# hyperconnect/TC-ResNet

Hardware: AMD Instinct MI355X
Metric: utterances/sec (1 s@16 kHz) TCResNet8-1.0 forward (higher is better)
Workload: dtype f32; 1 GPU; TCResNet8-1.0 eval forward, waveform->softmax, batch 4096/GPU, 49x40 MFCC (40/20 ms, FFT 1024), 12 classes; global_batch=4096, parallelism=dp1 (utterance shards, no collective)

## Files before the change

include/tcresnet_hip.h:

```cpp
#ifndef TCRESNET_HIP_H
#define TCRESNET_HIP_H

#include <stddef.h>
#include <stdint.h>

#ifdef __cplusplus
extern "C" {
#endif

#define TCR_ABI_VERSION 3
#define TCR_HALO 4
#define TCR_MAX_BLOCKS 16

typedef enum tcr_status {
    TCR_OK = 0,
    TCR_ERR_ARG = -1,
    TCR_ERR_HIP = -2,
    TCR_ERR_WORKSPACE = -3
} tcr_status;

int tcr_abi_version(void);
const char* tcr_last_error(void);
static inline int tcr_padded_len(int t) { return t + 2 * TCR_HALO; }

// ... 507 lines not shown
       TCR_TUNE_NET_SMALL = 27,
       TCR_TUNE_PW_POS = 28,
       TCR_TUNE_BN_APPLY = 29,
       TCR_TUNE_DW_DGRAD = 30,
       TCR_TUNE_DW_WGRAD = 31,
       TCR_TUNE_DW_FWD = 32,
       TCR_TUNE_WGRAD_PIPE = 33,
       TCR_TUNE_COMPOSE_RUN = 34,
       TCR_TUNE_COUNT = 35 };
int tcr_tune(int knob, int value);

int tcr_fused_deal_run(int nrt, int nt16, int nw, int wave, int* out3);

int tcr_fused_tm_taps(int k, int stride, int tin, int pad_lo, int tile, int* out2);
int tcr_fused_tm_deal(int k, int stride, int cin, int cout, int tin, int pad_lo, int nw, int wave, unsigned* jobs, int cap, int* mfma);
int tcr_net_fused_plan(const tcr_net* net, int batch, int* out, int cap);

void* tcr_internal_stream(int idx, void* caller_stream);

#ifdef __cplusplus
}
#endif
#endif
```

tc-resnet_amd/_lib.py:

```python
from __future__ import annotations

import ctypes as C
import os
from typing import Optional

HALO = 4
MAX_BLOCKS = 16
GRID_TILE = 256
MINE_TILE = 256
MINE_RADIUS_MAX = 2560
COMPOSE_TILE = 2048
REVERB_TILE = 4096
REVERB_STAGE = 1024
REVERB_TAPS_MAX = 16384
PHRASE_TILE = 256
PHRASE_MAX = 64
PHRASE_MAX_WORDS = 8
PHRASE_PRODUCT, PHRASE_MIN = 0, 1
DTW_MAX_TEMPLATES = 64
DTW_MAX_FEATURES = 64
ABI_VERSION = 3
_HERE = os.path.dirname(os.path.abspath(__file__))
HIP_LIB_PATH = os.path.join(_HERE, "lib", "libtcresnet_hip.so")

# ... 51 lines not shown
class TensorInfo(C.Structure):
    _fields_ = [("name", C.c_char * 96), ("kind", C.c_int32), ("arena", C.c_int32), ("offset", C.c_int64),
                ("size", C.c_int64), ("shape", C.c_int32 * 4), ("rank", C.c_int32)]


_P = C.c_void_p
_DTW_TABLES = (C.c_int, _P, _P, C.c_int, _P, _P, C.POINTER(DtwCfg))
_PROTOTYPES = {
    "tcr_abi_version": (C.c_int, []),
    "tcr_last_error": (C.c_char_p, []),
    "tcr_kernel_name": (C.c_char_p, [C.c_int]),
    "tcr_tune": (C.c_int, [C.c_int, C.c_int]),
    "tcr_fused_deal_run": (C.c_int, [C.c_int, C.c_int, C.c_int, C.c_int, C.POINTER(C.c_int)]),
    "tcr_fused_tm_taps": (C.c_int, [C.c_int, C.c_int, C.c_int, C.c_int, C.c_int, C.POINTER(C.c_int)]),
    "tcr_fused_tm_deal": (C.c_int, [C.c_int] * 8 + [C.POINTER(C.c_uint), C.c_int, C.POINTER(C.c_int)]),
    "tcr_net_fused_plan": (C.c_int, [_P, C.c_int, C.POINTER(C.c_int), C.c_int]),
    "tcr_internal_stream": (_P, [C.c_int, _P]),
    "tcr_frontend_resolve": (C.c_int, [C.POINTER(FrontendCfg)]),
    "tcr_frontend_plan_bytes": (C.c_size_t, [C.POINTER(FrontendCfg)]),
    "tcr_frontend_plan_init": (C.c_int, [C.POINTER(FrontendCfg), _P]),
    "tcr_frontend_plan_mel_matrix": (C.c_int, [C.POINTER(FrontendCfg), _P, _P]),
    "tcr_frontend_plan_dct_matrix": (C.c_int, [C.POINTER(FrontendCfg), _P, _P]),
    "tcr_frontend_fwd": (C.c_int, [C.POINTER(FrontendCfg), _P, _P, C.c_int, _P, _P]),
    "tcr_frontend_fwd_rounds": (C.c_int, [C.POINTER(FrontendCfg), _P, _P, C.c_int, _P, C.c_int, _P]),
    "tcr_features_to_planar": (C.c_int, [_P, C.c_int, C.c_int, C.c_int, _P, _P]),
    "tcr_features_from_planar": (C.c_int, [_P, C.c_int, C.c_int, C.c_int, _P, _P]),
    "tcr_tcresnet_create": (C.c_int, [C.POINTER(TCResNetCfg), C.POINTER(_P)]),
    "tcr_net_destroy": (None, [_P]),
    "tcr_net_param_floats": (C.c_int64, [_P]),
    "tcr_net_decay_floats": (C.c_int64, [_P]),
# ... 223 lines not shown
```

tc-resnet_amd/csrc/fused.hip:

```cpp
#include <cstdint>

#include "kernels.h"

namespace tcr {

typedef float f32x4 __attribute__((ext_vector_type(4)));
typedef float f32x2 __attribute__((ext_vector_type(2)));

__device__ __forceinline__ f32x4 buf_load_f32x4(buf_rsrc rs, unsigned lane_off_bytes, unsigned uniform_off_bytes) {
#if __has_builtin(__builtin_amdgcn_raw_buffer_load_b128)
    return __builtin_bit_cast(f32x4, __builtin_amdgcn_raw_buffer_load_b128(rs, (int)lane_off_bytes, (int)uniform_off_bytes, 0));
#else
    return (f32x4){buf_load_f32(rs, lane_off_bytes, uniform_off_bytes), buf_load_f32(rs, lane_off_bytes, uniform_off_bytes + 4u),
                   buf_load_f32(rs, lane_off_bytes, uniform_off_bytes + 8u), buf_load_f32(rs, lane_off_bytes, uniform_off_bytes + 12u)};
#endif
}
__device__ __forceinline__ f32x2 buf_load_f32x2(buf_rsrc rs, unsigned lane_off_bytes, unsigned uniform_off_bytes) {
#if __has_builtin(__builtin_amdgcn_raw_buffer_load_b64)
    return __builtin_bit_cast(f32x2, __builtin_amdgcn_raw_buffer_load_b64(rs, (int)lane_off_bytes, (int)uniform_off_bytes, 0));
#else
    return (f32x2){buf_load_f32(rs, lane_off_bytes, uniform_off_bytes), buf_load_f32(rs, lane_off_bytes, uniform_off_bytes + 4u)};
#endif
}

// ... 203 lines not shown
            for (int reg = 0; reg < 4; ++reg) {
                const int co = m * 16 + q * 4 + reg;
                if (co >= COUT) continue;
                float v = fmaf(ac[reg], sc[reg], sh[reg]);
                if (res) v = fmaxf(v + res[g * res_sz + co * TPO + kHalo + t], 0.f);
                else if (L.relu) v = fmaxf(v, 0.f);
                float* dst = yout + g * out_sz + co * TPO + kHalo + t;
                dst[0] = v;
                if (t == 0) { dst[-4] = 0.f; dst[-3] = 0.f; dst[-2] = 0.f; dst[-1] = 0.f; }
                if (t == TOUT - 1) { dst[1] = 0.f; dst[2] = 0.f; dst[3] = 0.f; dst[4] = 0.f; }
            }
        }
    }
}

template <int K, int S, int CIN, int COUT, int TIN, bool HAS_RES, int NTJ, bool WLDS, int AHEAD = 0, bool TM = false, int OCS = 0, bool IMG = false>
__device__ __forceinline__ void fused_job_s(const FusedArgs& a, const FusedLayer& L, const float* __restrict__ xin, const int in_sz,
                                            float* yout, const float* res, const float* w, const int npos, const int m, const int (&cc)[NTJ],
                                            const int r, const int q, const int jlo = 0, const int jhi = K - 1, const int wio = 0) {
    constexpr int TOUT = (TIN + S - 1) / S;
    constexpr int PADT = ((TOUT - 1) * S + K - TIN) > 0 ? ((TOUT - 1) * S + K - TIN) : 0;
    constexpr int PADLO = PADT / 2;
    constexpr int TPI = TM ? fused_tm_pitch(TIN, true, S) : TIN + 2 * kHalo;
    constexpr int TPO = TM ? fused_tm_pitch(TOUT, OCS != 0, OCS) : TOUT + 2 * kHalo;
    constexpr int TPR = TM ? fused_tm_pitch(TOUT, false, 0) : TPO;
    constexpr int JS = TM ? kTmGroup : 1;
    constexpr int C4 = CIN / 4;
    constexpr int WSTEP = 4 * COUT, XSTEP = 4 * TPI;
    const int out_sz = L.out_sz;
    const int res_sz = L.res_sz;
    const int ja = TM ? jlo : 0, jb = TM ? jhi : K - 1;
    int gg[NTJ], tt[NTJ];
    const float* xp[NTJ];
#pragma unroll
    for (int nt = 0; nt < NTJ; ++nt) {
        if constexpr (TM) {
            const int half = (TOUT % 2 == 1 && cc[nt] == TOUT / 2) ? 0 : (r >> 3);
            gg[nt] = half * 8 + min(r & 7, npos - 1);
            tt[nt] = cc[nt] * 16;
            xp[nt] = xin + q * TPI + (S == 1 ? gg[nt] : 2 * gg[nt] - (gg[nt] & 7)) + tt[nt] * S + kTmGroup * (kHalo - PADLO);
        } else {
        const int p = min(cc[nt], npos - 1);
        gg[nt] = p / TOUT;
        tt[nt] = p - gg[nt] * TOUT;
        xp[nt] = xin + gg[nt] * in_sz + q * TPI + tt[nt] * S + kHalo - PADLO;
        }
    }
    const float* wp = w + q * COUT + min(m * 16 + r, COUT - 1);
    static_assert(COUT % 4 == 0, "a lane's four output channels are valid or invalid together");
    const int cob = min(m * 16 + q * 4, COUT - 4);
    const buf_rsrc sr = make_rsrc(a.ss);
    const unsigned sl = (unsigned)cob * 4u;
    float sc[4], sh[4];
    if constexpr (IMG) {
        const f32x4 vs = buf_load_f32x4(sr, sl, (unsigned)L.ss_off * 4u), vh = buf_load_f32x4(sr, sl, (unsigned)(L.ss_off + L.c_pad) * 4u);
#pragma unroll
        for (int reg = 0; reg < 4; ++reg) { sc[reg] = vs[reg]; sh[reg] = vh[reg]; }
    } else {
#pragma unroll
    for (int reg = 0; reg < 4; ++reg) {
        sc[reg] = buf_load_f32(sr, sl, (unsigned)(L.ss_off + reg) * 4u);
        sh[reg] = buf_load_f32(sr, sl, (unsigned)(L.ss_off + L.c_pad + reg) * 4u);
    }
    }
    const buf_rsrc ir = make_rsrc(IMG ? a.wimg : a.params);
    const unsigned il = (unsigned)(q * 16 + r);
    const unsigned io = (unsigned)(kWimgHeader + wio + m * (K * C4 * 64)) * 4u;
    constexpr unsigned kTapBytes = (unsigned)(C4 * 64) * 4u;
    f32x4 acc[NTJ];
#pragma unroll
    for (int nt = 0; nt < NTJ; ++nt) acc[nt] = (f32x4){0.f, 0.f, 0.f, 0.f};
    if constexpr (AHEAD == 1) {
        const buf_rsrc wr = make_rsrc(a.params);
        const unsigned wl = (unsigned)(q * COUT + min(m * 16 + r, COUT - 1)) * 4u;
        const unsigned wo = (unsigned)L.w_off * 4u;
        float w0[C4], w1[C4];
        if constexpr (IMG) wimg_load<C4, 0, C4>(ir, il, io + (unsigned)ja * kTapBytes, w0);
        else {
#pragma unroll
        for (int c4 = 0; c4 < C4; ++c4) w0[c4] = buf_load_f32(wr, wl, wo + (unsigned)((ja * C4 + c4) * WSTEP) * 4u);
        }
        auto tap = [&](const int j, const float (&wu)[C4], float (&wf)[C4], const bool fill) {
            TCR_WHATIF_PRIO(32768, 2);
            if (fill && !(TCR_WHATIF(4096) && (!TCR_WHATIF(65536) || (S == 2 && CIN == 24 && COUT == 32)))) {
                if constexpr (IMG) wimg_load<C4, 0, C4>(ir, il, io + (unsigned)(j + 1) * kTapBytes, wf);
                else {
#pragma unroll
                for (int c4 = 0; c4 < C4; ++c4) wf[c4] = buf_load_f32(wr, wl, wo + (unsigned)(((j + 1) * C4 + c4) * WSTEP) * 4u);
                }
            }
            float b[NTJ][C4];
            if (TCR_WHATIF(8192) && j > 0) {
#pragma unroll
                for (int c4 = 0; c4 < C4; ++c4)
#pragma unroll
                    for (int nt = 0; nt < NTJ; ++nt) b[nt][c4] = wu[c4] + (float)nt;
            } else {
#pragma unroll
            for (int c4 = 0; c4 < C4; ++c4)
#pragma unroll
                for (int nt = 0; nt < NTJ; ++nt) b[nt][c4] = xp[nt][c4 * XSTEP + JS * j];
            }
            __builtin_amdgcn_sched_barrier(0);
            TCR_WHATIF_PRIO(16384, 2);
            TCR_WHATIF_PRIO(32768, 0);
#pragma unroll
            for (int c4 = 0; c4 < C4; ++c4)
#pragma unroll
                for (int nt = 0; nt < NTJ; ++nt) acc[nt] = TCR_MFMA(wu[c4], b[nt][c4], acc[nt]);
            TCR_WHATIF_PRIO(16384, 0);
        };
        if constexpr (TM) {
            int j = ja;
#pragma unroll 1
            for (; j + 2 <= jb; j += 2) {
                tap(j, w0, w1, true);
                tap(j + 1, w1, w0, true);
            }
            if (j == jb) {
                tap(j, w0, w1, false);
            } else {
                tap(j, w0, w1, true);
                tap(j + 1, w1, w0, false);
            }
// ... 38 lines not shown
    wfill_b(ja);
    constexpr int kTapUnroll = WLDS ? K : 1;
#pragma unroll kTapUnroll
    for (int j = ja; j <= jb; ++j) {
        const int jn = TCR_WHATIF(2) ? 0 : min(j + 1, jb);
        const int jx = TCR_WHATIF(4) ? 0 : JS * j;
        {
            float b[NTJ][H0 > 0 ? H0 : 1];
#pragma unroll
            for (int c4 = 0; c4 < H0; ++c4)
#pragma unroll
                for (int nt = 0; nt < NTJ; ++nt) b[nt][c4] = xp[nt][c4 * XSTEP + jx];
#pragma unroll
            for (int c4 = 0; c4 < H0; ++c4)
#pragma unroll
                for (int nt = 0; nt < NTJ; ++nt) acc[nt] = TCR_MFMA(wa[c4], b[nt][c4], acc[nt]);
            wfill_a(jn);
        }
        {
            float b[NTJ][H1];
#pragma unroll
            for (int c4 = 0; c4 < H1; ++c4)
#pragma unroll
                for (int nt = 0; nt < NTJ; ++nt) b[nt][c4] = xp[nt][(H0 + c4) * XSTEP + jx];
#pragma unroll
            for (int c4 = 0; c4 < H1; ++c4)
#pragma unroll
                for (int nt = 0; nt < NTJ; ++nt) acc[nt] = TCR_MFMA(wb[c4], b[nt][c4], acc[nt]);
            wfill_b(jn);
        }
    }
    }
    const int dump = a.buf_off[2] + a.group * a.buf_sz[2] + (q * 16 + r) - a.buf_off[L.out_buf];
    const float lo = L.relu ? 0.f : -3.4e38f;
    const bool cv = COUT % 16 == 0 || m * 16 + q * 4 < COUT;
    float rv[NTJ][4];
    if (HAS_RES) {
#pragma unroll
        for (int nt = 0; nt < NTJ; ++nt) {
            const int rb = TM ? cob * TPR + tt[nt] + gg[nt] : gg[nt] * res_sz + cob * TPO + kHalo + tt[nt];
#pragma unroll
            for (int reg = 0; reg < 4; ++reg) rv[nt][reg] = res[rb + reg * TPR];
        }
    }
#pragma unroll
    for (int nt = 0; nt < NTJ; ++nt) {
        const bool ok = (TM ? 2 * cc[nt] + (r >> 3) < TOUT && (r & 7) < npos : cc[nt] < npos) && cv && !TCR_WHATIF(32);
        const f32x4 ac = acc[nt];
        float* po = yout + (ok ? (TM ? tt[nt] + r + (OCS != 0 ? kTmGroup * kHalo : 0) : gg[nt] * out_sz + kHalo + tt[nt]) + cob * TPO : dump);
        const int pitch = ok ? TPO : 0;
#pragma unroll
        for (int reg = 0; reg < 4; ++reg) {
            float v = fmaf(ac[reg], sc[reg], sh[reg]);
            if (HAS_RES) v = fmaxf(v + rv[nt][reg], 0.f);
            else v = fmaxf(v, lo);
            *po = v;
            po += pitch;
        }
    }
}

template <int NW, int K, int S, int CIN, int COUT, int TIN, bool HAS_RES, int NTJ = 2, bool WLDS = false>
__device__ __forceinline__ void fused_layer_s(const FusedArgs& a, const FusedLayer& L, const float* __restrict__ xin, const int in_sz,
                                              float* lds, const int ng, const int wave, const int r_in, const int q_in,
                                              const int w_lds = 0) {
    const int oz = opaque_zero();
    const int r = r_in + oz, q = q_in + oz;
    constexpr int TOUT = (TIN + S - 1) / S;
    constexpr int NRT = (COUT + 15) / 16;
    constexpr int JP = 16 * NTJ;
    static_assert(CIN % 4 == 0, "channel quads");
    static_assert(NTJ == 1 || NTJ == 2 || NTJ == 4, "one, two or four 16-position tiles per job");
    float* yout = lds + a.buf_off[L.out_buf];
// ... 9 lines not shown
        for (int nt = 0; nt < NTJ; ++nt) cc[nt] = (IL && NTJ > 1) ? cp * JP + 32 * (nt >> 1) + 2 * r + (nt & 1) : cp * JP + 16 * nt + r;
        fused_job_s<K, S, CIN, COUT, TIN, HAS_RES, NTJ, WLDS>(a, L, xin, in_sz, yout, res, w, npos, m, cc, r, q);
    }
}

template <int NT, int COUT, int TOUT, int PITCH>
__device__ __forceinline__ void fused_zero_halo_tm(float* yout, const int tid_in) {
    if (TCR_WHATIF(1024)) return;
    const int tid = tid_in + opaque_zero();
    for (int i = tid; i < COUT * 16; i += NT) {
        float4* p = reinterpret_cast<float4*>(yout + (i >> 4) * PITCH + ((i & 8) ? kTmGroup * (kHalo + TOUT) : 0) + 4 * (i & 7));
        *p = make_float4(0.f, 0.f, 0.f, 0.f);
    }
}

template <int NW, int K, int S, int CIN, int COUT, int TIN, bool HAS_RES, int OCS, int AHEAD, bool IMG = false>
__device__ __forceinline__ void fused_layer_tm(const FusedArgs& a, const FusedLayer& L, float* lds, const int ng, const int wave, const int r_in, const int q_in, const int wio = 0) {
    constexpr int TOUT = (TIN + S - 1) / S;
    constexpr int PADT = ((TOUT - 1) * S + K - TIN) > 0 ? ((TOUT - 1) * S + K - TIN) : 0;
    static constexpr FusedTmDeal deal = fused_tm_deal(K, S, CIN, COUT, TIN, PADT / 2, NW);
    static_assert(fused_tm_deal_fits(deal, NW), "a wave's jobs exceed the deal's table (kTmMaxJobs)");
    float* yout = lds + a.buf_off[L.out_buf];
    if constexpr (OCS != 0) fused_zero_halo_tm<NW * 64, COUT, TOUT, fused_tm_pitch(TOUT, true, OCS)>(yout, (int)threadIdx.x);
    const int oz = opaque_zero();
    const int r = r_in + oz, q = q_in + oz;
    const float* xin = lds + a.buf_off[L.in_buf];
    const float* res = L.res_buf >= 0 ? lds + a.buf_off[L.res_buf] : nullptr;
    const float* w = a.params + L.w_off;
    const int n = deal.n[wave];
    for (int i = 0; i < n; ++i) {
        const unsigned jw = deal.job[wave][i];
        const int m = (int)(jw & 15u), c = (int)(jw >> 4 & 63u), lo = (int)(jw >> 11 & 15u), hi = (int)(jw >> 15 & 15u);
        if (jw >> 10 & 1u) {
            const int cc[2] = {c, c + 1};
            fused_job_s<K, S, CIN, COUT, TIN, HAS_RES, 2, false, AHEAD, true, OCS, IMG>(a, L, xin, 0, yout, res, w, ng, m, cc, r, q, lo, hi, wio);
        } else {
            const int cc[1] = {c};
            fused_job_s<K, S, CIN, COUT, TIN, HAS_RES, 1, false, AHEAD, true, OCS, IMG>(a, L, xin, 0, yout, res, w, ng, m, cc, r, q, lo, hi, wio);
        }
    }
}

template <int NW, int K, int S, int CIN, int COUT, int TIN, bool HAS_RES, int AHEAD = 0>
__device__ __forceinline__ void fused_layer_u(const FusedArgs& a, const FusedLayer& L, const float* __restrict__ xin, const int in_sz,
                                              float* lds, const int ng, const int wave, const int r_in, const int q_in) {
    const int oz = opaque_zero();
    const int r = r_in + oz, q = q_in + oz;
    constexpr int TOUT = (TIN + S - 1) / S;
    constexpr int NRT = (COUT + 15) / 16;
    constexpr bool IL = S == 1;
    float* yout = lds + a.buf_off[L.out_buf];
    const float* res = L.res_buf >= 0 ? lds + a.buf_off[L.res_buf] : nullptr;
    const int npos = ng * TOUT;
// ... 363 lines not shown
    }
}

struct Tc8Shape { int k, stride, cin, cout; };
__host__ __device__ constexpr Tc8Shape tc8_shape(const int li) {
    constexpr Tc8Shape shape[10] = {{3, 1, 40, 16}, {1, 2, 16, 24}, {9, 2, 16, 24}, {9, 1, 24, 24}, {1, 2, 24, 32},
                                    {9, 2, 24, 32}, {9, 1, 32, 32}, {1, 2, 32, 48}, {9, 2, 32, 48}, {9, 1, 48, 48}};
    return shape[li];
}
__host__ __device__ constexpr int tc8_wimg_off(const int li) {
    int n = 0;
    for (int i = 0; i < li && i < 10; ++i) n += wimg_layer_floats(tc8_shape(i).k, tc8_shape(i).cin, tc8_shape(i).cout);
    return n;
}

template <int NW, int T0, int WD, int NTJ0 = 2, bool TM = false>
__global__ __launch_bounds__(NW * 64) TCR_WAVES_PER_SIMD_4 void net_fused_tc8_kernel(const FusedArgs a) {
    constexpr bool IMG = false;
#include "fused_tc8_walk.inc"
}
template <int NW, int T0, int WD, int NTJ0, bool TM, bool IMG>
__device__ __forceinline__ void net_fused_tc8_walk(const FusedArgs& a) {
#include "fused_tc8_walk.inc"
}
template <int NW, int T0, int WD, int NTJ0, bool TM, bool WIMG>
__global__ __launch_bounds__(NW * 64) TCR_WAVES_PER_SIMD_4 void net_fused_tc8_kernel(const FusedArgs a) {
    static_assert(TM && WIMG, "the instance with a weight image is the time-major one");
    if (wimg_present(a)) net_fused_tc8_walk<NW, T0, WD, NTJ0, TM, true>(a);
    else net_fused_tc8_walk<NW, T0, WD, NTJ0, TM, false>(a);
}

template <int NW>
__device__ __forceinline__ void small_stage_weights(const float* __restrict__ src, int n_floats, float* dst, int wave, int lane) {
    for (int c0 = wave * 256; c0 < n_floats; c0 += NW * 256) {
        const int c = c0 + 4 * lane;
        if (c < n_floats) glds16(src + c, dst + c0);
    }
}

template <int NW, int T0>
__global__ __launch_bounds__(NW * 64) void net_small_tc8_kernel(const FusedArgs a, const int wa_off, const int wb_off) {
    constexpr int NT = NW * 64;
    constexpr int T1 = (T0 + 1) / 2, T2 = (T1 + 1) / 2, T3 = (T2 + 1) / 2;
    float* lds = reinterpret_cast<float*>(dyn_lds());
// ... 131 lines not shown
                                     {9, 1, 48, 48}, {9, 1, 48, 48}, {9, 1, 48, 48}, {1, 2, 48, 72}, {9, 2, 48, 72}, {9, 1, 72, 72}, {9, 1, 72, 72}, {9, 1, 72, 72}};
    if (a.n_layers != 16 || !a.in_global || a.in_c != 40) return 0;
    const int t0 = a.layer[0].tin;
    if (t0 != 49 && t0 != 98) return 0;
    int t = t0;
    for (int i = 0; i < 16; ++i) {
        const FusedLayer& L = a.layer[i];
        if (L.k != shape[i][0] || L.stride != shape[i][1] || L.cin != shape[i][2] || L.cout != shape[i][3] || L.tin != t) return 0;
        if (i == 2 || i == 7 || i == 12) t = (t + 1) / 2;
    }
    return t0;
}

static int fused_tc8_frames(const FusedArgs& a);
bool fused_tmajor_applies(const FusedArgs& a, const int waves) {
    return (tune_get(TCR_TUNE_NET_FUSED) == 0 || tune_get(TCR_TUNE_NET_FUSED) == 13) && a.group == kTmGroup && waves == 8 && a.nc == 12 && fused_tc8_frames(a) == 49;
}
static bool fused_tmajor_pitches_agree(const FusedArgs& a) {
    for (int i = 0; i < a.n_layers; ++i) {
        const FusedLayer& L = a.layer[i];
        const int ocs = (L.k == 1 || i == a.n_layers - 1) ? 0 : (L.stride == 2 ? 1 : 2);
        if (L.out_sz != fused_tm_pitch(L.tout, ocs != 0, ocs)) return false;
        if (i > 0 && L.in_sz != fused_tm_pitch(L.tin, true, L.stride)) return false;
        if (L.res_buf >= 0 && L.res_sz != fused_tm_pitch(L.tout, false, 0)) return false;
        if (L.pad_lo != (L.k == 9 ? 4 : L.k == 3 ? 1 : 0)) return false;
    }
    return a.feat_sz == fused_tm_pitch(a.feat_t, false, 0);
}

static int fused_tc8_frames(const FusedArgs& a) {
    if (a.n_layers != 10 || !a.in_global || a.in_c != 40) return 0;
// ... 221 lines not shown
    }
    const bool r2 = tune_get(TCR_TUNE_NET_FUSED) == 4;
    const bool j2 = tune_get(TCR_TUNE_NET_FUSED) == 8;
    const bool ju = tune_get(TCR_TUNE_NET_FUSED) == 9;
    const bool j4 = tune_get(TCR_TUNE_NET_FUSED) == 5;
    const bool jl = tune_get(TCR_TUNE_NET_FUSED) == 10;
    const bool jr = tune_get(TCR_TUNE_NET_FUSED) == 11;
#define TCR_FS(NW_, T_) if (tc8 == T_ && waves == NW_) kern = r2 ? net_fused_tc8_kernel<NW_, T_, -1> : (j4 ? net_fused_tc8_kernel<NW_, T_, 0, 4> : (ju ? net_fused_tc8_kernel<NW_, T_, 0, 0> : (j2 ? net_fused_tc8_kernel<NW_, T_, 0, 2> : ((jr || (T_ == 49 && !jl)) ? net_fused_tc8_kernel<NW_, T_, 0, 6> : net_fused_tc8_kernel<NW_, T_, 0, 3>))));
    TCR_FS(4, 49) TCR_FS(8, 49) TCR_FS(16, 49) TCR_FS(4, 98) TCR_FS(8, 98) TCR_FS(16, 98)
#undef TCR_FS
    if (a.tmajor) {
        if (!fused_tmajor_applies(a, waves) || !fused_tmajor_pitches_agree(a)) { set_error("fused kernel: time-major plan without its kernel instance"); return TCR_ERR_ARG; }
        constexpr int kImg = tc8_wimg_off(10);
        if (a.wimg_floats != kImg) { set_error("fused kernel: the plan's weight image has %d floats, the kernel's %d", a.wimg_floats, kImg); return TCR_ERR_ARG; }
        if (a.wimg && reinterpret_cast<uintptr_t>(a.wimg) % 16 != 0) { set_error("fused kernel: the frozen table's weight image is not on a 16-byte boundary"); return TCR_ERR_ARG; }
        kern = tune_get(TCR_TUNE_NET_FUSED) == 13 ? net_fused_tc8_kernel<8, 49, 0, 6, true> : net_fused_tc8_kernel<8, 49, 0, 6, true, true>;
    }
    const int tc14 = (kern || tune_get(TCR_TUNE_NET_FUSED) == 3 || tune_get(TCR_TUNE_NET_FUSED) == 4) ? 0 : fused_tc14w_frames(a);
#define TCR_F14(NW_, T_) if (tc14 == T_ && waves == NW_) kern = ju ? net_fused_tc14w_kernel<NW_, T_, 0> : (j2 ? net_fused_tc14w_kernel<NW_, T_, 2> : net_fused_tc14w_kernel<NW_, T_, 13>);
    TCR_F14(8, 49) TCR_F14(16, 49) TCR_F14(8, 98) TCR_F14(16, 98)
#undef TCR_F14
    if (kern) ring = 0;
#define TCR_FK(NW_, R_) if (!kern && waves == NW_ && ring == R_) kern = net_fused_kernel<NW_, R_>;
    TCR_FK(4, 4) TCR_FK(4, 8) TCR_FK(4, 16) TCR_FK(8, 4) TCR_FK(8, 8) TCR_FK(8, 16) TCR_FK(16, 4) TCR_FK(16, 8) TCR_FK(16, 16)
#undef TCR_FK
    if (!kern) { set_error("fused kernel: no instantiation for %d waves / ring %d", waves, ring); return TCR_ERR_ARG; }
    if (lds_bytes > 64 * 1024) {
        if (hipFuncSetAttribute(reinterpret_cast<const void*>(kern), hipFuncAttributeMaxDynamicSharedMemorySize, (int)lds_bytes) != hipSuccess) {
            (void)hipGetLastError();
            return 1;
        }
// ... 44 lines not shown

extern "C" int tcr_fused_tm_deal(int k, int stride, int cin, int cout, int tin, int pad_lo, int nw, int wave, unsigned* jobs, int cap, int* mfma) {
    if (!jobs || k < 1 || stride < 1 || cin < 4 || cout < 1 || cout > 256 || tin < 1 || tin > 126 || (nw != 4 && nw != 8 && nw != 16) || wave < 0 || wave >= nw || cap < tcr::kTmMaxJobs) {
        tcr::set_error("tcr_fused_tm_deal: bad arguments");
        return TCR_ERR_ARG;
    }
    const int tout = (tin + stride - 1) / stride;
    if (((cout + 15) / 16) * ((tout + 1) / 2) > nw * tcr::kTmMaxJobs) { tcr::set_error("tcr_fused_tm_deal: more jobs than the table holds"); return TCR_ERR_ARG; }
    const tcr::FusedTmDeal d = tcr::fused_tm_deal(k, stride, cin, cout, tin, pad_lo, nw);
    if (d.n[wave] > tcr::kTmMaxJobs) { tcr::set_error("tcr_fused_tm_deal: more jobs than the table holds"); return TCR_ERR_ARG; }
    for (int i = 0; i < d.n[wave]; ++i) jobs[i] = d.job[wave][i];
    if (mfma) *mfma = d.mfma;
    return d.n[wave];
}

extern "C" int tcr_fused_deal_run(int nrt, int nt16, int nw, int wave, int* out3) {
    if (!out3 || nrt < 1 || nt16 < 0 || nw < nrt || nw % nrt != 0 || wave < 0 || wave >= nw) {
        tcr::set_error("tcr_fused_deal_run: bad arguments (%d row tiles, %d column tiles, wave %d of %d)", nrt, nt16, wave, nw);
        return TCR_ERR_ARG;
    }
    const tcr::FusedRun run = tcr::fused_deal_run(nrt, nt16, nw, wave);
    out3[0] = run.m; out3[1] = run.c0; out3[2] = run.c1;
    return TCR_OK;
}
```

tc-resnet_amd/csrc/fused_tc8_walk.inc:

```
    constexpr int NT = NW * 64;
    constexpr int T1 = (T0 + 1) / 2, T2 = (T1 + 1) / 2;
    float* lds = reinterpret_cast<float*>(dyn_lds());
    const int tid = threadIdx.x;
    const int lane = tid & 63;
    const int wave = __builtin_amdgcn_readfirstlane(tid >> 6);
    const int r = lane & 15, q = lane >> 4;
    const int row = a.in_c * a.in_tp;
#if TCR_FUSED_WHATIF & 2048
    long long ts[14];
    int nts = 0;
#define TCR_TC8_BARRIER do { __syncthreads(); ts[nts++] = (long long)__builtin_readcyclecounter(); } while (0)
#elif TCR_FUSED_WHATIF & 8
#define TCR_TC8_BARRIER ((void)0)
#else
#define TCR_TC8_BARRIER __syncthreads()
#endif
    constexpr bool RES = WD >= 0 && NTJ0 == 6;
    constexpr int NTJU = RES ? 3 : NTJ0;
#define TCR_TC8_OCS(LI, K_, S_) ((K_ == 1 || LI == 9) ? 0 : (S_ == 2 ? 1 : 2))
#define TCR_TC8_WIO(LI) (IMG ? tc8_wimg_off(LI) : 0)
#define TCR_TC8(LI, K_, S_, CI_, CO_, T_) do { const FusedLayer& L_ = TCR_LAYER_ROW(WD >= 0, LI); \
        static_assert(tc8_shape(LI).k == K_ && tc8_shape(LI).stride == S_ && tc8_shape(LI).cin == CI_ && tc8_shape(LI).cout == CO_, "layer LI runs with row LI's shape (tc8_shape)"); \
        if constexpr (TM) fused_layer_tm<NW, K_, S_, CI_, CO_, T_, (LI == 3 || LI == 6 || LI == 9), TCR_TC8_OCS(LI, K_, S_), ((K_ == 9 && CI_ <= 32) ? 1 : 0), IMG>(a, L_, lds, ng, wave, r, q, TCR_TC8_WIO(LI)); \
        else fused_layer_sel<NW, K_, S_, CI_, CO_, T_, WD, (LI == 3 || LI == 6 || LI == 9), (K_ != 1 && LI != 9), ((LI >= 1 && LI <= 3 && NTJU == 4) ? 4 : (((NTJU == 0 || NTJU == 3) && K_ == 9) ? NTJU : 2))>(a, L_, lds + a.buf_off[L_.in_buf], L_.in_sz, lds, ng, wave, r, q); } while (0)
#define TCR_TC8_R(LI, S_, CI_, CO_, T_, WS_) do { const FusedLayer& L_ = TCR_LAYER_ROW(true, LI); \
        if constexpr (TM) fused_zero_halo_tm<NT, CO_, (T_ + S_ - 1) / S_, fused_tm_pitch((T_ + S_ - 1) / S_, true, TCR_TC8_OCS(LI, 9, S_))>(lds + a.buf_off[L_.out_buf], tid); \
        else fused_zero_halo<NT, CO_, (T_ + S_ - 1) / S_>(lds + a.buf_off[L_.out_buf], L_.out_sz, ng, tid); \
        fused_layer_r<NW, 9, S_, CI_, CO_, T_, (LI == 3), TM, TCR_TC8_OCS(LI, 9, S_), IMG>(a, L_, lds + a.buf_off[L_.in_buf], L_.in_sz, lds, ng, wave, r, q, WS_); } while (0)
    for (int grp = blockIdx.x; grp < (TCR_WHATIF(512) ? 0 : a.n_groups); grp += gridDim.x) {
        const int n0 = grp * a.group;
        const int ng = min(a.group, a.batch - n0);
#if TCR_FUSED_WHATIF & 2048
        nts = 0;
        ts[nts++] = (long long)__builtin_readcyclecounter();
#endif
        if constexpr (WD < 0) fused_layer_sel<NW, 3, 1, 40, 16, T0, WD, false>(a, a.layer[0], a.feat + (size_t)n0 * row, row, lds, ng, wave, r, q);
        else if (!TCR_WHATIF(64)) {
            const FusedLayer& L0 = TCR_LAYER_ROW(true, 0);
// ... 53 lines not shown
```

tc-resnet_amd/csrc/kernels.h:

```cpp
#pragma once
#include "tcr_common.h"

namespace tcr {

enum ConvEpilogue { EPI_RAW = 0, EPI_AFFINE = 1 };

struct ConvArgs {
    const float* x;
    const float* w;
    float* y;
    const float* scale;
    const float* shift;
    const float* res;
    int npos;
    int cin, cout;
    int tpi, tout, tpo;
    int xoff;
    int relu;
    int ostride, ooff;
    const float* add;
    const float* add_mask;
    int add_bcast;
};

// ... 189 lines not shown
        int best = -1;
        for (int i = 0; i < nj; ++i) if (!used[i] && (best < 0 || cost[i] > cost[best])) best = i;
        used[best] = true;
        int s = 0;
        for (int i = 1; i < 4 && i < nw; ++i) if (sload[i] < sload[s]) s = i;
        int w = s;
        for (int i = s + 4; i < nw; i += 4) if (wload[i] < wload[w]) w = i;
        if (d.n[w] < kTmMaxJobs) d.job[w][d.n[w]] = words[best];
        ++d.n[w];
        wload[w] += cost[best];
        sload[s] += cost[best];
    }
    return d;
}

struct FusedRun { int m, c0, c1; };
__host__ __device__ inline FusedRun fused_deal_run(const int nrt, const int nt16, const int nw, const int wave) {
    const int wpt = nw / nrt;
    const int m = wave / wpt, l = wave - m * wpt;
    const int per = nt16 / wpt, extra = nt16 - per * wpt;
    const int rank = (l + wpt - (m * extra) % wpt) % wpt;
    const int c0 = rank * per + (rank < extra ? rank : extra);
    return FusedRun{m, c0, c0 + per + (rank < extra ? 1 : 0)};
}

__host__ __device__ constexpr bool fused_tm_deal_fits(const FusedTmDeal& d, const int nw) {
    for (int w = 0; w < nw; ++w) if (d.n[w] > kTmMaxJobs) return false;
    return true;
}

// ... 342 lines not shown
```

Baseline: 20.63 million utterances/s.

## Span all output-channel row tiles per job in early tc8 layers

Adds a row-spanning job mode to the time-major fused tc8 kernel. For layers 1 and 2, each job computes every 16-channel output tile for a time column, so each activation B fragment loaded per tap is reused across all row tiles. A new deal function distributes these larger jobs across waves, and the default kernel selection now uses this mode. The trade is more accumulator and weight registers per lane and fewer, coarser jobs, which may unbalance waves or reduce occupancy.

Result: no change. 20.62 million utterances/s (-0.0%).

```diff
diff --git a/include/tcresnet_hip.h b/include/tcresnet_hip.h
--- a/include/tcresnet_hip.h
+++ b/include/tcresnet_hip.h
@@ -545,6 +545,7 @@
 
 int tcr_fused_tm_taps(int k, int stride, int tin, int pad_lo, int tile, int* out2);
 int tcr_fused_tm_deal(int k, int stride, int cin, int cout, int tin, int pad_lo, int nw, int wave, unsigned* jobs, int cap, int* mfma);
+int tcr_fused_tm_deal_rows(int k, int stride, int cin, int cout, int tin, int pad_lo, int nw, int ntj, int wave, unsigned* jobs, int cap, int* mfma);
 int tcr_net_fused_plan(const tcr_net* net, int batch, int* out, int cap);
 
 void* tcr_internal_stream(int idx, void* caller_stream);
diff --git a/tc-resnet_amd/_lib.py b/tc-resnet_amd/_lib.py
--- a/tc-resnet_amd/_lib.py
+++ b/tc-resnet_amd/_lib.py
@@ -89,6 +89,7 @@
     "tcr_fused_deal_run": (C.c_int, [C.c_int, C.c_int, C.c_int, C.c_int, C.POINTER(C.c_int)]),
     "tcr_fused_tm_taps": (C.c_int, [C.c_int, C.c_int, C.c_int, C.c_int, C.c_int, C.POINTER(C.c_int)]),
     "tcr_fused_tm_deal": (C.c_int, [C.c_int] * 8 + [C.POINTER(C.c_uint), C.c_int, C.POINTER(C.c_int)]),
+    "tcr_fused_tm_deal_rows": (C.c_int, [C.c_int] * 9 + [C.POINTER(C.c_uint), C.c_int, C.POINTER(C.c_int)]),
     "tcr_net_fused_plan": (C.c_int, [_P, C.c_int, C.POINTER(C.c_int), C.c_int]),
     "tcr_internal_stream": (_P, [C.c_int, _P]),
     "tcr_frontend_resolve": (C.c_int, [C.POINTER(FrontendCfg)]),
diff --git a/tc-resnet_amd/csrc/fused.hip b/tc-resnet_amd/csrc/fused.hip
--- a/tc-resnet_amd/csrc/fused.hip
+++ b/tc-resnet_amd/csrc/fused.hip
@@ -241,7 +241,7 @@
     }
 }
 
-template <int K, int S, int CIN, int COUT, int TIN, bool HAS_RES, int NTJ, bool WLDS, int AHEAD = 0, bool TM = false, int OCS = 0, bool IMG = false>
+template <int K, int S, int CIN, int COUT, int TIN, bool HAS_RES, int NTJ, bool WLDS, int AHEAD = 0, bool TM = false, int OCS = 0, bool IMG = false, int MT = 1>
 __device__ __forceinline__ void fused_job_s(const FusedArgs& a, const FusedLayer& L, const float* __restrict__ xin, const int in_sz,
                                             float* yout, const float* res, const float* w, const int npos, const int m, const int (&cc)[NTJ],
                                             const int r, const int q, const int jlo = 0, const int jhi = K - 1, const int wio = 0) {
@@ -254,6 +254,7 @@
     constexpr int JS = TM ? kTmGroup : 1;
     constexpr int C4 = CIN / 4;
     constexpr int WSTEP = 4 * COUT, XSTEP = 4 * TPI;
+    static_assert(MT == 1 || (TM && AHEAD == 1 && !WLDS), "row-spanning jobs: the time-major walk with a tap of weight lookahead");
     const int out_sz = L.out_sz;
     const int res_sz = L.res_sz;
     const int ja = TM ? jlo : 0, jb = TM ? jhi : K - 1;
@@ -275,53 +276,61 @@
     }
     const float* wp = w + q * COUT + min(m * 16 + r, COUT - 1);
     static_assert(COUT % 4 == 0, "a lane's four output channels are valid or invalid together");
-    const int cob = min(m * 16 + q * 4, COUT - 4);
     const buf_rsrc sr = make_rsrc(a.ss);
-    const unsigned sl = (unsigned)cob * 4u;
-    float sc[4], sh[4];
+    int cob[MT];
+    float sc[MT][4], sh[MT][4];
+#pragma unroll
+    for (int mt = 0; mt < MT; ++mt) {
+    cob[mt] = min((m + mt) * 16 + q * 4, COUT - 4);
+    const unsigned sl = (unsigned)cob[mt] * 4u;
     if constexpr (IMG) {
         const f32x4 vs = buf_load_f32x4(sr, sl, (unsigned)L.ss_off * 4u), vh = buf_load_f32x4(sr, sl, (unsigned)(L.ss_off + L.c_pad) * 4u);
 #pragma unroll
-        for (int reg = 0; reg < 4; ++reg) { sc[reg] = vs[reg]; sh[reg] = vh[reg]; }
+        for (int reg = 0; reg < 4; ++reg) { sc[mt][reg] = vs[reg]; sh[mt][reg] = vh[reg]; }
     } else {
 #pragma unroll
     for (int reg = 0; reg < 4; ++reg) {
-        sc[reg] = buf_load_f32(sr, sl, (unsigned)(L.ss_off + reg) * 4u);
-        sh[reg] = buf_load_f32(sr, sl, (unsigned)(L.ss_off + L.c_pad + reg) * 4u);
+        sc[mt][reg] = buf_load_f32(sr, sl, (unsigned)(L.ss_off + reg) * 4u);
+        sh[mt][reg] = buf_load_f32(sr, sl, (unsigned)(L.ss_off + L.c_pad + reg) * 4u);
+    }
     }
     }
     const buf_rsrc ir = make_rsrc(IMG ? a.wimg : a.params);
     const unsigned il = (unsigned)(q * 16 + r);
     const unsigned io = (unsigned)(kWimgHeader + wio + m * (K * C4 * 64)) * 4u;
-    constexpr unsigned kTapBytes = (unsigned)(C4 * 64) * 4u;
-    f32x4 acc[NTJ];
-#pragma unroll
-    for (int nt = 0; nt < NTJ; ++nt) acc[nt] = (f32x4){0.f, 0.f, 0.f, 0.f};
+    constexpr unsigned kTapBytes = (unsigned)(C4 * 64) * 4u, kRowBytes = (unsigned)K * kTapBytes;
+    f32x4 acc[NTJ][MT];
+#pragma unroll
+    for (int nt = 0; nt < NTJ; ++nt)
+#pragma unroll
+        for (int mt = 0; mt < MT; ++mt) acc[nt][mt] = (f32x4){0.f, 0.f, 0.f, 0.f};
     if constexpr (AHEAD == 1) {
         const buf_rsrc wr = make_rsrc(a.params);
-        const unsigned wl = (unsigned)(q * COUT + min(m * 16 + r, COUT - 1)) * 4u;
+        unsigned wl[MT];
+#pragma unroll
+        for (int mt = 0; mt < MT; ++mt) wl[mt] = (unsigned)(q * COUT + min((m + mt) * 16 + r, COUT - 1)) * 4u;
         const unsigned wo = (unsigned)L.w_off * 4u;
-        float w0[C4], w1[C4];
-        if constexpr (IMG) wimg_load<C4, 0, C4>(ir, il, io + (unsigned)ja * kTapBytes, w0);
-        else {
-#pragma unroll
-        for (int c4 = 0; c4 < C4; ++c4) w0[c4] = buf_load_f32(wr, wl, wo + (unsigned)((ja * C4 + c4) * WSTEP) * 4u);
-        }
-        auto tap = [&](const int j, const float (&wu)[C4], float (&wf)[C4], const bool fill) {
+        float w0[MT][C4], w1[MT][C4];
+        auto wreq = [&](const int j, float (&wf)[MT][C4]) {
+#pragma unroll
+            for (int mt = 0; mt < MT; ++mt) {
+                if constexpr (IMG) wimg_load<C4, 0, C4>(ir, il, io + (unsigned)mt * kRowBytes + (unsigned)j * kTapBytes, wf[mt]);
+                else {
+#pragma unroll
+                for (int c4 = 0; c4 < C4; ++c4) wf[mt][c4] = buf_load_f32(wr, wl[mt], wo + (unsigned)((j * C4 + c4) * WSTEP) * 4u);
+                }
+            }
+        };
+        wreq(ja, w0);
+        auto tap = [&](const int j, const float (&wu)[MT][C4], float (&wf)[MT][C4], const bool fill) {
             TCR_WHATIF_PRIO(32768, 2);
-            if (fill && !(TCR_WHATIF(4096) && (!TCR_WHATIF(65536) || (S == 2 && CIN == 24 && COUT == 32)))) {
-                if constexpr (IMG) wimg_load<C4, 0, C4>(ir, il, io + (unsigned)(j + 1) * kTapBytes, wf);
-                else {
-#pragma unroll
-                for (int c4 = 0; c4 < C4; ++c4) wf[c4] = buf_load_f32(wr, wl, wo + (unsigned)(((j + 1) * C4 + c4) * WSTEP) * 4u);
-                }
-            }
+            if (fill && !(TCR_WHATIF(4096) && (!TCR_WHATIF(65536) || (S == 2 && CIN == 24 && COUT == 32)))) wreq(j + 1, wf);
             float b[NTJ][C4];
             if (TCR_WHATIF(8192) && j > 0) {
 #pragma unroll
                 for (int c4 = 0; c4 < C4; ++c4)
 #pragma unroll
-                    for (int nt = 0; nt < NTJ; ++nt) b[nt][c4] = wu[c4] + (float)nt;
+                    for (int nt = 0; nt < NTJ; ++nt) b[nt][c4] = wu[0][c4] + (float)nt;
             } else {
 #pragma unroll
             for (int c4 = 0; c4 < C4; ++c4)
@@ -334,7 +343,9 @@
 #pragma unroll
             for (int c4 = 0; c4 < C4; ++c4)
 #pragma unroll
-                for (int nt = 0; nt < NTJ; ++nt) acc[nt] = TCR_MFMA(wu[c4], b[nt][c4], acc[nt]);
+                for (int nt = 0; nt < NTJ; ++nt)
+#pragma unroll
+                    for (int mt = 0; mt < MT; ++mt) acc[nt][mt] = TCR_MFMA(wu[mt][c4], b[nt][c4], acc[nt][mt]);
             TCR_WHATIF_PRIO(16384, 0);
         };
         if constexpr (TM) {
@@ -403,7 +414,7 @@
 #pragma unroll
             for (int c4 = 0; c4 < H0; ++c4)
 #pragma unroll
-                for (int nt = 0; nt < NTJ; ++nt) acc[nt] = TCR_MFMA(wa[c4], b[nt][c4], acc[nt]);
+                for (int nt = 0; nt < NTJ; ++nt) acc[nt][0] = TCR_MFMA(wa[c4], b[nt][c4], acc[nt][0]);
             wfill_a(jn);
         }
         {
@@ -415,19 +426,21 @@
 #pragma unroll
             for (int c4 = 0; c4 < H1; ++c4)
 #pragma unroll
-                for (int nt = 0; nt < NTJ; ++nt) acc[nt] = TCR_MFMA(wb[c4], b[nt][c4], acc[nt]);
+                for (int nt = 0; nt < NTJ; ++nt) acc[nt][0] = TCR_MFMA(wb[c4], b[nt][c4], acc[nt][0]);
             wfill_b(jn);
         }
     }
     }
     const int dump = a.buf_off[2] + a.group * a.buf_sz[2] + (q * 16 + r) - a.buf_off[L.out_buf];
     const float lo = L.relu ? 0.f : -3.4e38f;
-    const bool cv = COUT % 16 == 0 || m * 16 + q * 4 < COUT;
+#pragma unroll
+    for (int mt = 0; mt < MT; ++mt) {
+    const bool cv = COUT % 16 == 0 || (m + mt) * 16 + q * 4 < COUT;
     float rv[NTJ][4];
     if (HAS_RES) {
 #pragma unroll
         for (int nt = 0; nt < NTJ; ++nt) {
-            const int rb = TM ? cob * TPR + tt[nt] + gg[nt] : gg[nt] * res_sz + cob * TPO + kHalo + tt[nt];
+            const int rb = TM ? cob[mt] * TPR + tt[nt] + gg[nt] : gg[nt] * res_sz + cob[mt] * TPO + kHalo + tt[nt];
 #pragma unroll
             for (int reg = 0; reg < 4; ++reg) rv[nt][reg] = res[rb + reg * TPR];
         }
@@ -435,17 +448,18 @@
 #pragma unroll
     for (int nt = 0; nt < NTJ; ++nt) {
         const bool ok = (TM ? 2 * cc[nt] + (r >> 3) < TOUT && (r & 7) < npos : cc[nt] < npos) && cv && !TCR_WHATIF(32);
-        const f32x4 ac = acc[nt];
-        float* po = yout + (ok ? (TM ? tt[nt] + r + (OCS != 0 ? kTmGroup * kHalo : 0) : gg[nt] * out_sz + kHalo + tt[nt]) + cob * TPO : dump);
+        const f32x4 ac = acc[nt][mt];
+        float* po = yout + (ok ? (TM ? tt[nt] + r + (OCS != 0 ? kTmGroup * kHalo : 0) : gg[nt] * out_sz + kHalo + tt[nt]) + cob[mt] * TPO : dump);
         const int pitch = ok ? TPO : 0;
 #pragma unroll
         for (int reg = 0; reg < 4; ++reg) {
-            float v = fmaf(ac[reg], sc[reg], sh[reg]);
+            float v = fmaf(ac[reg], sc[mt][reg], sh[mt][reg]);
             if (HAS_RES) v = fmaxf(v + rv[nt][reg], 0.f);
             else v = fmaxf(v, lo);
             *po = v;
             po += pitch;
         }
+    }
     }
 }
 
@@ -485,11 +499,13 @@
     }
 }
 
-template <int NW, int K, int S, int CIN, int COUT, int TIN, bool HAS_RES, int OCS, int AHEAD, bool IMG = false>
+template <int NW, int K, int S, int CIN, int COUT, int TIN, bool HAS_RES, int OCS, int AHEAD, bool IMG = false, int ROWS = 0>
 __device__ __forceinline__ void fused_layer_tm(const FusedArgs& a, const FusedLayer& L, float* lds, const int ng, const int wave, const int r_in, const int q_in, const int wio = 0) {
     constexpr int TOUT = (TIN + S - 1) / S;
     constexpr int PADT = ((TOUT - 1) * S + K - TIN) > 0 ? ((TOUT - 1) * S + K - TIN) : 0;
-    static constexpr FusedTmDeal deal = fused_tm_deal(K, S, CIN, COUT, TIN, PADT / 2, NW);
+    constexpr int MT = ROWS != 0 ? (COUT + 15) / 16 : 1;
+    static_assert(ROWS == 0 || AHEAD == 1, "row-spanning jobs walk with a tap of weight lookahead");
+    static constexpr FusedTmDeal deal = ROWS != 0 ? fused_tm_deal_rows(K, S, CIN, COUT, TIN, PADT / 2, NW, ROWS) : fused_tm_deal(K, S, CIN, COUT, TIN, PADT / 2, NW);
     static_assert(fused_tm_deal_fits(deal, NW), "a wave's jobs exceed the deal's table (kTmMaxJobs)");
     float* yout = lds + a.buf_off[L.out_buf];
     if constexpr (OCS != 0) fused_zero_halo_tm<NW * 64, COUT, TOUT, fused_tm_pitch(TOUT, true, OCS)>(yout, (int)threadIdx.x);
@@ -502,12 +518,12 @@
     for (int i = 0; i < n; ++i) {
         const unsigned jw = deal.job[wave][i];
         const int m = (int)(jw & 15u), c = (int)(jw >> 4 & 63u), lo = (int)(jw >> 11 & 15u), hi = (int)(jw >> 15 & 15u);
-        if (jw >> 10 & 1u) {
+        if (ROWS != 1 && (jw >> 10 & 1u)) {
             const int cc[2] = {c, c + 1};
-            fused_job_s<K, S, CIN, COUT, TIN, HAS_RES, 2, false, AHEAD, true, OCS, IMG>(a, L, xin, 0, yout, res, w, ng, m, cc, r, q, lo, hi, wio);
+            fused_job_s<K, S, CIN, COUT, TIN, HAS_RES, 2, false, AHEAD, true, OCS, IMG, MT>(a, L, xin, 0, yout, res, w, ng, m, cc, r, q, lo, hi, wio);
         } else {
             const int cc[1] = {c};
-            fused_job_s<K, S, CIN, COUT, TIN, HAS_RES, 1, false, AHEAD, true, OCS, IMG>(a, L, xin, 0, yout, res, w, ng, m, cc, r, q, lo, hi, wio);
+            fused_job_s<K, S, CIN, COUT, TIN, HAS_RES, 1, false, AHEAD, true, OCS, IMG, MT>(a, L, xin, 0, yout, res, w, ng, m, cc, r, q, lo, hi, wio);
         }
     }
 }
@@ -901,20 +917,25 @@
     return n;
 }
 
+__host__ __device__ constexpr int tc8_rows_policy(const int rs, const int li) {
+    return (rs == 1 && (li == 1 || li == 2)) ? 1 : 0;
+}
+
 template <int NW, int T0, int WD, int NTJ0 = 2, bool TM = false>
 __global__ __launch_bounds__(NW * 64) TCR_WAVES_PER_SIMD_4 void net_fused_tc8_kernel(const FusedArgs a) {
     constexpr bool IMG = false;
+    constexpr int RS = 0;
 #include "fused_tc8_walk.inc"
 }
-template <int NW, int T0, int WD, int NTJ0, bool TM, bool IMG>
+template <int NW, int T0, int WD, int NTJ0, bool TM, bool IMG, int RS>
 __device__ __forceinline__ void net_fused_tc8_walk(const FusedArgs& a) {
 #include "fused_tc8_walk.inc"
 }
-template <int NW, int T0, int WD, int NTJ0, bool TM, bool WIMG>
+template <int NW, int T0, int WD, int NTJ0, bool TM, bool WIMG, int RS = 0>
 __global__ __launch_bounds__(NW * 64) TCR_WAVES_PER_SIMD_4 void net_fused_tc8_kernel(const FusedArgs a) {
     static_assert(TM && WIMG, "the instance with a weight image is the time-major one");
-    if (wimg_present(a)) net_fused_tc8_walk<NW, T0, WD, NTJ0, TM, true>(a);
-    else net_fused_tc8_walk<NW, T0, WD, NTJ0, TM, false>(a);
+    if (wimg_present(a)) net_fused_tc8_walk<NW, T0, WD, NTJ0, TM, true, RS>(a);
+    else net_fused_tc8_walk<NW, T0, WD, NTJ0, TM, false, RS>(a);
 }
 
 template <int NW>
@@ -1076,7 +1097,7 @@
 
 static int fused_tc8_frames(const FusedArgs& a);
 bool fused_tmajor_applies(const FusedArgs& a, const int waves) {
-    return (tune_get(TCR_TUNE_NET_FUSED) == 0 || tune_get(TCR_TUNE_NET_FUSED) == 13) && a.group == kTmGroup && waves == 8 && a.nc == 12 && fused_tc8_frames(a) == 49;
+    return (tune_get(TCR_TUNE_NET_FUSED) == 0 || tune_get(TCR_TUNE_NET_FUSED) == 13 || tune_get(TCR_TUNE_NET_FUSED) == 14) && a.group == kTmGroup && waves == 8 && a.nc == 12 && fused_tc8_frames(a) == 49;
 }
 static bool fused_tmajor_pitches_agree(const FusedArgs& a) {
     for (int i = 0; i < a.n_layers; ++i) {
@@ -1328,7 +1349,8 @@
         constexpr int kImg = tc8_wimg_off(10);
         if (a.wimg_floats != kImg) { set_error("fused kernel: the plan's weight image has %d floats, the kernel's %d", a.wimg_floats, kImg); return TCR_ERR_ARG; }
         if (a.wimg && reinterpret_cast<uintptr_t>(a.wimg) % 16 != 0) { set_error("fused kernel: the frozen table's weight image is not on a 16-byte boundary"); return TCR_ERR_ARG; }
-        kern = tune_get(TCR_TUNE_NET_FUSED) == 13 ? net_fused_tc8_kernel<8, 49, 0, 6, true> : net_fused_tc8_kernel<8, 49, 0, 6, true, true>;
+        const int knob = tune_get(TCR_TUNE_NET_FUSED);
+        kern = knob == 13 ? net_fused_tc8_kernel<8, 49, 0, 6, true> : (knob == 14 ? net_fused_tc8_kernel<8, 49, 0, 6, true, true> : net_fused_tc8_kernel<8, 49, 0, 6, true, true, 1>);
     }
     const int tc14 = (kern || tune_get(TCR_TUNE_NET_FUSED) == 3 || tune_get(TCR_TUNE_NET_FUSED) == 4) ? 0 : fused_tc14w_frames(a);
 #define TCR_F14(NW_, T_) if (tc14 == T_ && waves == NW_) kern = ju ? net_fused_tc14w_kernel<NW_, T_, 0> : (j2 ? net_fused_tc14w_kernel<NW_, T_, 2> : net_fused_tc14w_kernel<NW_, T_, 13>);
@@ -1403,6 +1425,19 @@
     return d.n[wave];
 }
 
+extern "C" int tcr_fused_tm_deal_rows(int k, int stride, int cin, int cout, int tin, int pad_lo, int nw, int ntj, int wave, unsigned* jobs, int cap, int* mfma) {
+    if (!jobs || k < 1 || stride < 1 || cin < 4 || cout < 1 || cout > 256 || tin < 1 || tin > 126 || (nw != 4 && nw != 8 && nw != 16) || (ntj != 1 && ntj != 2) || wave < 0 ||
+        wave >= nw || cap < tcr::kTmMaxJobs) {
+        tcr::set_error("tcr_fused_tm_deal_rows: bad arguments");
+        return TCR_ERR_ARG;
+    }
+    const tcr::FusedTmDeal d = tcr::fused_tm_deal_rows(k, stride, cin, cout, tin, pad_lo, nw, ntj);
+    if (!tcr::fused_tm_deal_fits(d, nw)) { tcr::set_error("tcr_fused_tm_deal_rows: more jobs than the table holds"); return TCR_ERR_ARG; }
+    for (int i = 0; i < d.n[wave]; ++i) jobs[i] = d.job[wave][i];
+    if (mfma) *mfma = d.mfma;
+    return d.n[wave];
+}
+
 extern "C" int tcr_fused_deal_run(int nrt, int nt16, int nw, int wave, int* out3) {
     if (!out3 || nrt < 1 || nt16 < 0 || nw < nrt || nw % nrt != 0 || wave < 0 || wave >= nw) {
         tcr::set_error("tcr_fused_deal_run: bad arguments (%d row tiles, %d column tiles, wave %d of %d)", nrt, nt16, wave, nw);
diff --git a/tc-resnet_amd/csrc/fused_tc8_walk.inc b/tc-resnet_amd/csrc/fused_tc8_walk.inc
--- a/tc-resnet_amd/csrc/fused_tc8_walk.inc
+++ b/tc-resnet_amd/csrc/fused_tc8_walk.inc
@@ -21,7 +21,7 @@
 #define TCR_TC8_WIO(LI) (IMG ? tc8_wimg_off(LI) : 0)
 #define TCR_TC8(LI, K_, S_, CI_, CO_, T_) do { const FusedLayer& L_ = TCR_LAYER_ROW(WD >= 0, LI); \
         static_assert(tc8_shape(LI).k == K_ && tc8_shape(LI).stride == S_ && tc8_shape(LI).cin == CI_ && tc8_shape(LI).cout == CO_, "layer LI runs with row LI's shape (tc8_shape)"); \
-        if constexpr (TM) fused_layer_tm<NW, K_, S_, CI_, CO_, T_, (LI == 3 || LI == 6 || LI == 9), TCR_TC8_OCS(LI, K_, S_), ((K_ == 9 && CI_ <= 32) ? 1 : 0), IMG>(a, L_, lds, ng, wave, r, q, TCR_TC8_WIO(LI)); \
+        if constexpr (TM) fused_layer_tm<NW, K_, S_, CI_, CO_, T_, (LI == 3 || LI == 6 || LI == 9), TCR_TC8_OCS(LI, K_, S_), (((K_ == 9 && CI_ <= 32) || tc8_rows_policy(RS, LI) != 0) ? 1 : 0), IMG, tc8_rows_policy(RS, LI)>(a, L_, lds, ng, wave, r, q, TCR_TC8_WIO(LI)); \
         else fused_layer_sel<NW, K_, S_, CI_, CO_, T_, WD, (LI == 3 || LI == 6 || LI == 9), (K_ != 1 && LI != 9), ((LI >= 1 && LI <= 3 && NTJU == 4) ? 4 : (((NTJU == 0 || NTJU == 3) && K_ == 9) ? NTJU : 2))>(a, L_, lds + a.buf_off[L_.in_buf], L_.in_sz, lds, ng, wave, r, q); } while (0)
 #define TCR_TC8_R(LI, S_, CI_, CO_, T_, WS_) do { const FusedLayer& L_ = TCR_LAYER_ROW(true, LI); \
         if constexpr (TM) fused_zero_halo_tm<NT, CO_, (T_ + S_ - 1) / S_, fused_tm_pitch((T_ + S_ - 1) / S_, true, TCR_TC8_OCS(LI, 9, S_))>(lds + a.buf_off[L_.out_buf], tid); \
diff --git a/tc-resnet_amd/csrc/kernels.h b/tc-resnet_amd/csrc/kernels.h
--- a/tc-resnet_amd/csrc/kernels.h
+++ b/tc-resnet_amd/csrc/kernels.h
@@ -227,6 +227,44 @@
     return d;
 }
 
+__host__ __device__ constexpr FusedTmDeal fused_tm_deal_rows(const int k, const int stride, const int cin, const int cout, const int tin, const int pad_lo, const int nw,
+                                                             const int ntj) {
+    FusedTmDeal d{};
+    const int tout = (tin + stride - 1) / stride, nt16 = (tout + 1) / 2, nrt = (cout + 15) / 16;
+    unsigned words[64] = {};
+    int cost[64] = {};
+    int nj = 0;
+    for (int c = 0; c < nt16;) {
+        const FusedTaps t = fused_tm_taps(k, stride, tin, pad_lo, c);
+        bool pair = false;
+        if (ntj >= 2 && c + 1 < nt16) {
+            const FusedTaps u = fused_tm_taps(k, stride, tin, pad_lo, c + 1);
+            pair = u.lo == t.lo && u.hi == t.hi;
+        }
+        words[nj] = (unsigned)c << 4 | (pair ? 1u : 0u) << 10 | (unsigned)t.lo << 11 | (unsigned)t.hi << 15;
+        cost[nj] = (t.hi - t.lo + 1) * (cin / 4) * (pair ? 2 : 1) * nrt;
+        d.mfma += cost[nj];
+        ++nj;
+        c += pair ? 2 : 1;
+    }
+    int wload[16] = {}, sload[4] = {};
+    bool used[64] = {};
+    for (int it = 0; it < nj; ++it) {
+        int best = -1;
+        for (int i = 0; i < nj; ++i) if (!used[i] && (best < 0 || cost[i] > cost[best])) best = i;
+        used[best] = true;
+        int s = 0;
+        for (int i = 1; i < 4 && i < nw; ++i) if (sload[i] < sload[s]) s = i;
+        int w = s;
+        for (int i = s + 4; i < nw; i += 4) if (wload[i] < wload[w]) w = i;
+        if (d.n[w] < kTmMaxJobs) d.job[w][d.n[w]] = words[best];
+        ++d.n[w];
+        wload[w] += cost[best];
+        sload[s] += cost[best];
+    }
+    return d;
+}
+
 struct FusedRun { int m, c0, c1; };
 __host__ __device__ inline FusedRun fused_deal_run(const int nrt, const int nt16, const int nw, const int wave) {
     const int wpt = nw / nrt;
```
